# oleg-savchenko/jax_nbody_emulator_with_dj

Hardware: AMD Instinct MI355X
Metric: voxels/sec (disp+vel) on 512^3 box, ndiv=4 (higher is better)
Workload: dtype f32-equivalent: f16x3 split MFMA (3 f16 MFMAs per product, f32 accumulate)

## Files before the change

### jax_nbody_emulator_with_dj_amd/csrc/nbe_kernels_wino.h

```cpp

#ifndef NBE_EPI_MAX
#define NBE_EPI_MAX 1
#endif
#ifndef NBE_WINO_ZROW
#define NBE_WINO_ZROW 1
#endif
#ifndef NBE_WINO_ITEMREG
#define NBE_WINO_ITEMREG 1
#endif
#ifndef NBE_WINO_LOU
#define NBE_WINO_LOU (NBE_XF_F32 ? 0 : 1)
#endif
constexpr int NBE_MAX_WSTAGES = 32;
constexpr int NBE_MAX_WSKIP = 16;
constexpr float WINO_WSCALE = 16384.0f;
constexpr float WINO_WSCALE_F16 = 256.0f;

struct WinoSrc { const char* xa; const char* xb; long dxd; const char* w; long psb; float sb; int pad_; };

struct WinoKArgs {
    int H, W, Dv, Hv, Wv, Ho, Wo;
    int nchunk, cout_groups, flags, ntiles, tny, tnx;
    int zblock;
    float* y; float* dy; long out_pstride; int out_g0;
    const float* bias; const float* gout; const float* beta;
    const float* r; const float* dr; long res_pstride;
    float inv_scale;
    int nskip;
    long dws_delta;
    WinoSrc st[NBE_MAX_WSTAGES + NBE_MAX_WSKIP];
};

template <bool SKIP, bool NOVEL, bool F16 = false>
__global__ __launch_bounds__(512, 2) void conv_h3w_kernel(WinoKArgs a) {
    static_assert(!(F16 && NOVEL), "the float16 form has no displacement-only variant");
    typedef HGGeom<false> G;
    constexpr int NW = 8, CT = 64, TAPU = G::TAPU, WGU = G::WG, XBASE = G::XBASE, MT = 4, NT = 2, NTILE = 8;
    constexpr int ZROW = G::LDS_UNITS;
    f32x4* lds = lds_h3;
    const half8* L8 = (const half8*)lds_h3;
    half8* L8w = (half8*)lds_h3;
    const int tid = threadIdx.x;
    const int lane = tid & 63;
    const int wave = __builtin_amdgcn_readfirstlane(tid >> 6);
    const int c = lane & 15, q = lane >> 4, kh = q & 1, ks = q >> 1;

    const int nct = (a.cout_groups + 7) / 8;
    const int vt = xcd_tile(blockIdx.x, a.ntiles * nct);
    const int tile = vt / nct, ct = vt - tile * nct;
    const int npair = a.Dv >> 1;
    int zp, ty, tx;
    {
        const int zb = a.zblock;
        const int full = (npair / zb) * zb;
        const int per_blk = zb * a.tny * a.tnx;
        if (tile < (npair / zb) * per_blk) {
            const int blk = tile / per_blk, r = tile - blk * per_blk;
            const int zi = r % zb, tyx = r / zb;
            zp = blk * zb + zi; ty = tyx / a.tnx; tx = tyx - ty * a.tnx;
        } else {
            const int r = tile - (npair / zb) * per_blk, rem = npair - full;
            const int zi = r % rem, tyx = r / rem;
            zp = full + zi; ty = tyx / a.tnx; tx = tyx - ty * a.tnx;
        }
    }
    const int y0 = ty * (NOVEL ? 2 * HP_ROWS : HP_ROWS), x0 = tx * HP_COLS, z0 = 2 * zp;
    const int nst = 4 * a.nchunk;

    const long to = (((long)z0 * a.H + y0) * a.W + x0) * 16;
    const long wcm = (long)ct * nst * WGU * 16, wcs = (long)ct * a.nskip * TAPU * 16;

    struct Nxt { const char *xa, *xb, *w0; long dxd, psb; float sb; } nx;
    auto set_next = [&](int s) {
        const WinoSrc e = a.st[s];
        nx.xa = e.xa + to; nx.xb = e.xb + to; nx.dxd = e.dxd; nx.psb = e.psb; nx.w0 = e.w + (SKIP && s >= nst ? wcs : wcm); nx.sb = e.sb;
    };
    unsigned lane16 = (unsigned)lane << 4;
    asm volatile("" : "+v"(lane16));
    auto dma_w = [&](int buf, int t) {
        const int n = wave + NW * t;
        unsigned l16 = (unsigned)lane;
        if (NBE_WINO_ZROW && !F16) l16 = lane16;
        else asm volatile("v_lshlrev_b32 %0, 4, %0" : "+v"(l16));
        if (n < G::NWI) dma16s(nx.w0 + (long)n * 1024, l16, lds + buf * WGU + n * 64);
    };
    auto dma_raw = [&](int buf) {
        unsigned l16 = (unsigned)lane;
        asm volatile("v_lshlrev_b32 %0, 4, %0" : "+v"(l16));
        dma16s(nx.w0 + (wave < 4 ? 0 : a.dws_delta) + (long)(wave & 3) * 1024, l16, lds + buf * WGU + wave * 64);
#pragma unroll
        for (int t = 0; t < 6; ++t) {
            const int tensor = t / 3, n = wave + NW * (t % 3), pl = n / 6, k = n - 6 * pl;
            const int u = k * 64 + lane;
            const int uu = u < HP_PL ? u : HP_PL - 1;
            const int row = (uu * 241) >> 13, col = uu - row * HP_RS;
            if (u < HP_PL)
                dma16s(nx.xa + (tensor ? nx.dxd : 0) + (long)pl * nx.psb, (unsigned)(row * a.W + col) * 16u,
                       lds + XBASE + buf * HQ_XB + tensor * HQ_XT + pl * HQ_PP + k * 64);
        }
    };
    constexpr bool ITEMREG = NBE_WINO_ITEMREG && !F16;
    int it_uu[3] = {0, 0, 0};
    unsigned it_go[3] = {0u, 0u, 0u};
    if (ITEMREG) {
#pragma unroll
        for (int j = 0; j < 3; ++j) {
            const int u = ((wave + NW * j) % 6) * 64 + lane;
            it_uu[j] = u < HP_PL ? u : HP_PL - 1;
            const int row = (it_uu[j] * 241) >> 13, col = it_uu[j] - row * HP_RS;
            it_go[j] = (unsigned)(row * a.W + col) * 16u;
        }
#pragma unroll
        for (int j = 0; j < 3; ++j) asm volatile("" : "+v"(it_uu[j]), "+v"(it_go[j]));
    }
    auto item_unit = [&](int j, bool& valid) {
        if (ITEMREG) {
            valid = lane < HP_PL - ((wave + NW * j) % 6) * 64;
            return it_uu[j];
        }
        int l = lane;
        asm volatile("" : "+v"(l));
        const int u = ((wave + NW * j) % 6) * 64 + l;
        valid = u < HP_PL;
        return valid ? u : HP_PL - 1;
    };
    auto item_goff_j = [&](int j) {
        if (ITEMREG) return it_go[j];
        bool v;
        const int uu = item_unit(j, v);
        const int row = (uu * 241) >> 13, col = uu - row * HP_RS;
        return (unsigned)(row * a.W + col) * 16u;
    };
    typedef unsigned int u32x4 __attribute__((ext_vector_type(4)));
    struct Stg { half8 ah, al, bh, bl; float sb; };
    auto st_load = [&](int j, Stg& g) {
        const int n = wave + NW * j;
        const long po = ((n / 12) ? nx.dxd : 0) + (long)(((n % 12) / 6) * 2) * nx.psb;
        const char* pa = nx.xa + po;
        const char* pb = nx.xb + po;
        const unsigned go = item_goff_j(j);
        const __amdgpu_buffer_rsrc_t ra = __builtin_amdgcn_make_buffer_rsrc((void*)pa, 0, 0xffffffffu, 0x00027000);
        const __amdgpu_buffer_rsrc_t rb = __builtin_amdgcn_make_buffer_rsrc((void*)pb, 0, 0xffffffffu, 0x00027000);
        const unsigned pso = (unsigned)nx.psb;
        auto ld = [&](half8& d, __amdgpu_buffer_rsrc_t r, unsigned so) {
            const u32x4 v = __builtin_amdgcn_raw_buffer_load_b128(r, go, so, 0);
            d = __builtin_bit_cast(half8, v);
        };
        ld(g.ah, ra, 0); ld(g.al, ra, pso); ld(g.bh, rb, 0); ld(g.bl, rb, pso);
        g.sb = nx.sb;
    };
#if NBE_XF_F32
    struct Xf { u32x4 HI, LO; float t0, t1; unsigned h; };
    auto xf_step = [&](const Stg& g, Xf& x, int k) {
        const int r = k >> 2, m = k & 3;
        const unsigned AH = __builtin_bit_cast(u32x4, g.ah)[r], AL = __builtin_bit_cast(u32x4, g.al)[r];
        const unsigned BH = __builtin_bit_cast(u32x4, g.bh)[r], BL = __builtin_bit_cast(u32x4, g.bl)[r];
        const float inv = H3_INV, sinv = g.sb * H3_INV, sb = g.sb, k2048 = H3_SCALE;
        if (m == 0) {
            asm("v_fma_mix_f32 %0, %1, %2, %3 op_sel:[0,0,0] op_sel_hi:[1,0,1]" : "=v"(x.t0) : "v"(AL), "s"(inv), "v"(AH));
            asm("v_fma_mix_f32 %0, %1, %2, %0 op_sel:[0,0,0] op_sel_hi:[1,0,0]" : "+v"(x.t0) : "v"(BL), "s"(sinv));
            asm("v_fma_mix_f32 %0, %1, %2, %0 op_sel:[0,0,0] op_sel_hi:[1,0,0]" : "+v"(x.t0) : "v"(BH), "s"(sb));
        } else if (m == 1) {
            asm("v_fma_mix_f32 %0, %1, %2, %3 op_sel:[1,0,1] op_sel_hi:[1,0,1]" : "=v"(x.t1) : "v"(AL), "s"(inv), "v"(AH));
            asm("v_fma_mix_f32 %0, %1, %2, %0 op_sel:[1,0,0] op_sel_hi:[1,0,0]" : "+v"(x.t1) : "v"(BL), "s"(sinv));
            asm("v_fma_mix_f32 %0, %1, %2, %0 op_sel:[1,0,0] op_sel_hi:[1,0,0]" : "+v"(x.t1) : "v"(BH), "s"(sb));
        } else if (m == 2) {
            asm("v_cvt_pk_f16_f32 %0, %1, %2" : "=v"(x.h) : "v"(x.t0), "v"(x.t1));
            asm("v_fma_mix_f32 %0, %1, -1.0, %0 op_sel:[0,0,0] op_sel_hi:[1,0,0]" : "+v"(x.t0) : "v"(x.h));
            asm("v_fma_mix_f32 %0, %1, -1.0, %0 op_sel:[1,0,0] op_sel_hi:[1,0,0]" : "+v"(x.t1) : "v"(x.h));
        } else {
            unsigned l;
            asm("v_fma_mixlo_f16 %0, %1, %2, 0 op_sel_hi:[0,0,0]" : "=v"(l) : "v"(x.t0), "s"(k2048));
            asm("v_fma_mixhi_f16 %0, %1, %2, 0 op_sel_hi:[0,0,0]" : "+v"(l) : "v"(x.t1), "s"(k2048));
            x.HI[r] = x.h; x.LO[r] = l;
        }
    };
#else
    struct Xf { u32x4 HI, LO; unsigned s, bb, e1, e2, l1; };
    auto xf_step = [&](const Stg& g, Xf& x, int k) {
        const int r = k >> 2, m = k & 3;
        const unsigned AH = __builtin_bit_cast(u32x4, g.ah)[r], AL = __builtin_bit_cast(u32x4, g.al)[r];
        const unsigned BH = __builtin_bit_cast(u32x4, g.bh)[r], BL = __builtin_bit_cast(u32x4, g.bl)[r];
        const unsigned sbp = g.sb < 0.f ? 0xBC00BC00u : 0x3C003C00u, k2048 = 0x68006800u;
        if (F16) {
            if (m == 0) asm("v_pk_fma_f16 %0, %1, %2, %3" : "=v"(x.s) : "v"(BH), "s"(sbp), "v"(AH));
            else if (m == 1) asm("v_pk_fma_f16 %0, %1, %2, %3" : "=v"(x.l1) : "v"(BL), "s"(sbp), "v"(AL));
            else if (m == 3) { x.HI[r] = x.s; x.LO[r] = x.l1; }
            (void)k2048;
        } else
        if (m == 0) {
            asm("v_pk_fma_f16 %0, %1, %2, %3" : "=v"(x.s) : "v"(BH), "s"(sbp), "v"(AH));
            asm("v_pk_add_f16 %0, %1, %2 neg_lo:[0,1] neg_hi:[0,1]" : "=v"(x.bb) : "v"(x.s), "v"(AH));
        } else if (m == 1) {
            asm("v_pk_add_f16 %0, %1, %2 neg_lo:[0,1] neg_hi:[0,1]" : "=v"(x.e1) : "v"(x.s), "v"(x.bb));
            asm("v_pk_fma_f16 %0, %1, %2, %3 neg_lo:[0,0,1] neg_hi:[0,0,1]" : "=v"(x.e2) : "v"(BH), "s"(sbp), "v"(x.bb));
        } else if (m == 2) {
            asm("v_pk_add_f16 %0, %1, %2 neg_lo:[0,1] neg_hi:[0,1]" : "=v"(x.e1) : "v"(AH), "v"(x.e1));
            asm("v_pk_fma_f16 %0, %1, %2, %3" : "=v"(x.l1) : "v"(BL), "s"(sbp), "v"(AL));
        } else {
            unsigned err, l;
            asm("v_pk_add_f16 %0, %1, %2" : "=v"(err) : "v"(x.e1), "v"(x.e2));
#if NBE_WINO_LOU
            const unsigned kinv = 0x10001000u;
            asm("v_pk_fma_f16 %0, %1, %2, %3" : "=v"(l) : "v"(x.l1), "s"(kinv), "v"(err));
            (void)k2048;
#else
            asm("v_pk_fma_f16 %0, %1, %2, %3" : "=v"(l) : "v"(err), "s"(k2048), "v"(x.l1));
#endif
            x.HI[r] = x.s; x.LO[r] = l;
        }
    };
#endif
    auto st_write = [&](int j, int buf, const Xf& x) {
        bool valid;
        const int n = wave + NW * j;
        const int lo_ = XBASE + buf * HQ_XB + (n / 12) * HQ_XT + (((n % 12) / 6) * 2) * HQ_PP + item_unit(j, valid);
        if (valid) {
            L8w[lo_] = __builtin_bit_cast(half8, x.HI);
            L8w[lo_ + HQ_PP] = __builtin_bit_cast(half8, x.LO);
        }
    };
    auto st_store = [&](int j, int buf, Stg& g) {
        Xf x;
#pragma unroll
        for (int k = 0; k < 16; ++k) xf_step(g, x, k);
        st_write(j, buf, x);
    };

    f32x4 YA[NTILE], DA[NTILE], YB[NTILE], DB[NTILE];
#pragma unroll
    for (int t = 0; t < NTILE; ++t)
#pragma unroll
        for (int e = 0; e < 4; ++e) { YA[t][e] = 0.f; DA[t][e] = 0.f; YB[t][e] = 0.f; DB[t][e] = 0.f; }
    auto mm = [&](f32x4& acc, const half8& A, const half8& B) {
        asm("v_mfma_f32_16x16x32_f16 %0, %1, %2, %0" : "+a"(acc) : "v"(A), "v"(B));
    };
    auto mmz = [&](f32x4& acc, const half8& A, const half8& B) {
        asm("s_nop 1\n\tv_mfma_f32_16x16x32_f16 %0, %1, %2, %0" : "+a"(acc) : "v"(A), "v"(B));
    };

    const int rowp = wave;
    const int aP = (ks * 4 + 2 * kh) * CT + c;
    const int bB = (2 * kh) * HQ_PP + rowp * HP_RS + c;
    const int bP1 = bB + ks, bP32 = bB + 32 * ks;
    auto LA = [&](half8 (&r)[MT], int idx) {
#pragma unroll
        for (int mt = 0; mt < MT; ++mt) r[mt] = L8[idx + 16 * mt];
    };
    auto LB = [&](half8 (&r)[NT], int idx) {
#pragma unroll
        for (int nt = 0; nt < NT; ++nt) r[nt] = L8[idx + 16 * nt];
    };
    const _Float16 kInv = (_Float16)H3_INV;
#define SNAKE(i) ((((i) >> 1) & 1) ? ((i) ^ 1) : (i))
    auto nohook = [](int) {};
    auto MM8h = [&](f32x4 (&acc)[NTILE], const half8 (&A)[MT], const half8 (&B)[NT], int slot, int nb, bool px, bool zsel,
                    bool hooked, auto&& hook) {
#pragma unroll
        for (int i = 0; i < NTILE; ++i) {
            const int t = SNAKE(i);
            if (zsel && (i % NT) == 0) mmz(acc[t], A[t / NT], B[t % NT]); else
            mm(acc[t], A[t / NT], B[t % NT]);
            if (hooked) { hook(i); __builtin_amdgcn_sched_barrier(0); }
            if (slot >= 0 && (i % 4) == 3) {
                if (px) dma_w(nb, slot + i / 4);
                __builtin_amdgcn_sched_barrier(0);
            }
        }
    };
    auto MM8 = [&](f32x4 (&acc)[NTILE], const half8 (&A)[MT], const half8 (&B)[NT], int slot, int nb, bool px, bool zsel = false) {
        MM8h(acc, A, B, slot, nb, px, zsel, false, nohook);
    };
    auto MM8s = [&](f32x4 (&acc)[NTILE], half8 (&P)[MT], const half8 (&A)[MT], const half8 (&B)[NT], int slot, int nb, bool px) {
        P[0] = A[0] * kInv;
#pragma unroll
        for (int i = 0; i < NTILE; ++i) {
            const int t = SNAKE(i);
            if ((i % NT) == 0) { if (t / NT + 1 < MT) P[t / NT + 1] = A[t / NT + 1] * kInv; mmz(acc[t], P[t / NT], B[t % NT]); }
            else mm(acc[t], P[t / NT], B[t % NT]);
            if (slot >= 0 && (i % 4) == 3) {
                if (px) dma_w(nb, slot + i / 4);
                __builtin_amdgcn_sched_barrier(0);
            }
        }
    };
#define NBE_SB __builtin_amdgcn_sched_barrier(0)
    half8 wh[MT], wl[MT], wp[MT], xh[NT], xl[NT], dxh[NT], dxl[NT];
    auto pair = [&](f32x4 (&Y)[NTILE], f32x4 (&DY)[NTILE], int slot0, int nb, bool px, int wa, int xp,
                    auto&& preXl, auto&& preW, auto&& preXh, auto&& mid, bool hooked, auto&& hook, auto&& after3) {
        if (F16) {
            LB(dxh, xp + HQ_XT); LA(wl, wa + CT + aP);
            NBE_SB; MM8h(Y, wh, xh, slot0, nb, px, false, hooked, [&](int t) { hook(t); }); NBE_SB;
            LB(dxl, xp + HQ_XT + HQ_PP);
            NBE_SB; MM8h(Y, wl, xl, slot0 < 0 ? -1 : slot0 + 2, nb, px, false, hooked, [&](int t) { hook(8 + t); }); NBE_SB;
            after3();
            mid();
            preXl(); preXh();
            NBE_SB; MM8(DY, wh, dxh, slot0 < 0 ? -1 : slot0 + 4, nb, px); NBE_SB;
            preW();
            NBE_SB; MM8(DY, wl, dxl, -1, nb, px); NBE_SB;
            return;
        }
        LB(dxh, xp + HQ_XT);
#if NBE_WINO_LOU
        NBE_SB; MM8(Y, wh, xl, slot0, nb, px); NBE_SB;
#else
        NBE_SB; MM8s(Y, wp, wh, xl, slot0, nb, px); NBE_SB;
#endif
        LB(dxl, xp + HQ_XT + HQ_PP);
        NBE_SB; MM8h(Y, wh, xh, slot0 < 0 ? -1 : slot0 + 2, nb, px, false, hooked, [&](int t) { hook(t); }); NBE_SB;
        LA(wl, wa + CT + aP);
        NBE_SB; MM8h(DY, wh, dxh, slot0 < 0 ? -1 : slot0 + 4, nb, px, false, hooked, [&](int t) { hook(8 + t); }); NBE_SB;
        after3();
        mid();
#if NBE_WINO_LOU
        NBE_SB; MM8(DY, wh, dxl, -1, nb, px); NBE_SB;
#else
        NBE_SB; MM8(DY, wp, dxl, -1, nb, px); NBE_SB;
#endif
        preXl(); preW();
        NBE_SB; MM8(Y, wl, xh, -1, nb, px); NBE_SB;
        preXh();
        NBE_SB; MM8(DY, wl, dxh, -1, nb, px); NBE_SB;
    };

    constexpr int SH4 = HP_RS + 1, SH5 = HP_RS + 2, SH7 = 2 * HP_RS + 1;
    auto stage = [&](f32x4 (&Y)[NTILE], f32x4 (&DY)[NTILE], int s, auto nxt) {
        constexpr int NXT = decltype(nxt)::value;
        constexpr bool px = NXT == 1;
        const bool pre = px && s + 1 != 2 * a.nchunk;
        if (NXT) set_next(s + 1);
        int par = s & 1;
        asm volatile("" : "+s"(par));
        int nb = 1 - par;
        asm volatile("" : "+s"(nb));
        const int wb = par * WGU, xb = XBASE + par * HQ_XB;
        const int wbn = nb * WGU, xbn = XBASE + nb * HQ_XB;
        Stg g;
        Xf xf;
        auto hk = [&](int k) { xf_step(g, xf, k); };
        auto none = [] {};
        if (NXT == 2) dma_raw(nb);
        if (px) st_load(0, g);
        pair(Y, DY, 0, nb, px, wb, xb + bP1,
             [&] { LB(xl, xb + 2 + bP32 + HQ_PP); }, [&] { LA(wh, wb + 2 * TAPU + aP); }, [&] { LB(xh, xb + 2 + bP32); },
             none, false, nohook, none);
        half8 a1[MT], a2[MT], b1x[NT], b1d[NT];
        const int aS = wb + 4 * TAPU + (2 * kh + (F16 ? ks : 0)) * CT + c;
        const int bS = xb + (2 * kh + ks) * HQ_PP + rowp * HP_RS + c + SH4;
        pair(Y, DY, -1, nb, px, wb + 2 * TAPU, xb + 2 + bP32,
             [&] { LB(b1x, bS); }, [&] { LA(a1, aS); }, [&] { LB(b1d, bS + HQ_XT); }, none,
             px, hk, [&] { if (px) { st_write(0, nb, xf); st_load(1, g); } });
        const half8 zero = {0, 0, 0, 0, 0, 0, 0, 0};
        if (F16) {
            NBE_SB; MM8(Y, a1, b1x, -1, 0, false); NBE_SB;
            LB(xl, xb + SH5 + bP32 + HQ_PP); LB(xh, xb + SH5 + bP32); LA(wh, wb + 5 * TAPU + aP);
            NBE_SB; MM8(DY, a1, b1d, -1, 0, false); NBE_SB;
        } else {
#if NBE_WINO_LOU
        NBE_SB; MM8(Y, a1, b1x, -1, 0, false); NBE_SB;
#else
        {
            const _Float16 m1 = ks ? kInv : (_Float16)1.0f;
#pragma unroll
            for (int mt = 0; mt < MT; ++mt) a1[mt] = a1[mt] * m1;
        }
        NBE_SB; MM8(Y, a1, b1x, -1, 0, false, true); NBE_SB;
#endif
#if NBE_WINO_ZROW
        LA(a2, ks ? ZROW + c : aS + CT);
#else
        LA(a2, aS + CT);
#endif
        LB(xl, xb + SH5 + bP32 + HQ_PP);
        NBE_SB; MM8(DY, a1, b1d, -1, 0, false); NBE_SB;
        LB(xh, xb + SH5 + bP32); LA(wh, wb + 5 * TAPU + aP);
#if NBE_WINO_ZROW
        NBE_SB; MM8(Y, a2, b1x, -1, 0, false); NBE_SB;
#else
#pragma unroll
        for (int mt = 0; mt < MT; ++mt) a2[mt] = ks ? zero : a2[mt];
        NBE_SB; MM8(Y, a2, b1x, -1, 0, false, true); NBE_SB;
#endif
        MM8(DY, a2, b1d, -1, 0, false); NBE_SB;
        }
        pair(Y, DY, -1, nb, px, wb + 5 * TAPU, xb + SH5 + bP32,
             [&] { LB(xl, xb + SH7 + bP1 + HQ_PP); }, [&] { LA(wh, wb + 7 * TAPU + aP); }, [&] { LB(xh, xb + SH7 + bP1); },
             none, px, hk, [&] { if (px) { st_write(1, nb, xf); st_load(2, g); } });
        pair(Y, DY, -1, nb, px, wb + 7 * TAPU, xb + SH7 + bP1,
             [&] { if (pre) LB(xl, xbn + bP1 + HQ_PP); }, [&] { if (pre) LA(wh, wbn + aP); }, [&] { if (pre) LB(xh, xbn + bP1); },
             [&] { asm volatile("s_waitcnt vmcnt(0) lgkmcnt(0)\n\ts_barrier" ::: "memory"); },
             px, hk, [&] { if (px) st_write(2, nb, xf); });
    };

    auto raw_stage = [&](f32x4 (&Y)[NTILE], f32x4 (&DY)[NTILE], int s, bool px) {
        if (px) set_next(s + 1);
        int par = s & 1;
        asm volatile("" : "+s"(par));
        int nb = 1 - par;
        asm volatile("" : "+s"(nb));
        const int wb = par * WGU, xb = XBASE + par * HQ_XB;
        if (px) dma_raw(nb);
        half8 a1[MT], a2[MT], d1[MT], d2[MT], bx[NT], bd[NT];
        const half8 zero = {0, 0, 0, 0, 0, 0, 0, 0};
        const _Float16 m1 = ks ? kInv : (_Float16)1.0f;
        const int aS = wb + (2 * kh) * CT + c;
        const int bS = xb + (2 * kh + ks) * HQ_PP + rowp * HP_RS + c + SH4;
        if (F16) {
            const int aF = wb + (2 * kh + ks) * CT + c;
            LA(a1, aF); LB(bx, bS); LB(bd, bS + HQ_XT); LA(d1, aF + TAPU);
            NBE_SB; MM8(Y, a1, bx, -1, 0, false); NBE_SB;
            MM8(DY, a1, bd, -1, 0, false); NBE_SB;
            MM8(DY, d1, bx, -1, 0, false); NBE_SB;
            asm volatile("s_waitcnt vmcnt(0) lgkmcnt(0)\n\ts_barrier" ::: "memory");
            return;
        }
        LA(a1, aS); LB(bx, bS); LA(a2, aS + CT); LB(bd, bS + HQ_XT);
#pragma unroll
        for (int mt = 0; mt < MT; ++mt) a1[mt] = a1[mt] * m1;
        NBE_SB; MM8(Y, a1, bx, -1, 0, false, true); NBE_SB;
        if (!NOVEL) LA(d1, aS + TAPU);
#pragma unroll
        for (int mt = 0; mt < MT; ++mt) a2[mt] = ks ? zero : a2[mt];
        NBE_SB; MM8(Y, a2, bx, -1, 0, false, true); NBE_SB;
        if (!NOVEL) LA(d2, aS + TAPU + CT);
        if (NOVEL || !(a.flags & F_SKIP_NODX)) {
            NBE_SB; MM8(DY, a1, bd, -1, 0, false); NBE_SB;
            MM8(DY, a2, bd, -1, 0, false); NBE_SB;
        }
        if (!NOVEL) {
#pragma unroll
            for (int mt = 0; mt < MT; ++mt) { d1[mt] = d1[mt] * m1; d2[mt] = ks ? zero : d2[mt]; }
            NBE_SB; MM8(DY, d1, bx, -1, 0, false, true); NBE_SB;
            MM8(DY, d2, bx, -1, 0, false, true); NBE_SB;
        }
        asm volatile("s_waitcnt vmcnt(0) lgkmcnt(0)\n\ts_barrier" ::: "memory");
    };

    {
        if (NBE_WINO_ZROW && !F16 && tid < 64) L8w[ZROW + tid] = half8{0, 0, 0, 0, 0, 0, 0, 0};
        set_next(0);
#pragma unroll
        for (int k = 0; k < G::NWS; ++k) dma_w(0, k);
        {
            Stg g0, g1, g2;
            st_load(0, g0); st_load(1, g1); st_load(2, g2);
            st_store(0, 0, g0); st_store(1, 0, g1); st_store(2, 0, g2);
        }
        asm volatile("s_waitcnt vmcnt(0) lgkmcnt(0)" ::: "memory");
        __syncthreads();
        LA(wh, aP); LB(xl, XBASE + bP1 + HQ_PP); LB(xh, XBASE + bP1);
    }

    auto butterfly = [&] {
            asm volatile("s_nop 15\n\ts_nop 15" ::: "memory");
#pragma unroll
            for (int t = 0; t < NTILE; ++t) {
                f32x4 p, m;
#pragma unroll
                for (int e = 0; e < 4; ++e) { p[e] = acc_read(YA[t][e]); m[e] = acc_read(YB[t][e]); }
                YA[t] = p + m; YB[t] = p - m;
                asm volatile("" : "+a"(YA[t]), "+a"(YB[t]));
                __builtin_amdgcn_sched_barrier(0);
#pragma unroll
                for (int e = 0; e < 4; ++e) { p[e] = acc_read(DA[t][e]); m[e] = acc_read(DB[t][e]); }
                DA[t] = p + m; DB[t] = p - m;
                asm volatile("" : "+a"(DA[t]), "+a"(DB[t]));
                __builtin_amdgcn_sched_barrier(0);
            }
            asm volatile("s_nop 7" ::: "memory");
            LA(wh, aP); LB(xl, XBASE + bP1 + HQ_PP); LB(xh, XBASE + bP1);
    };
    const int npairs = 2 * a.nchunk;
    for (int s2 = 0; s2 + 1 < npairs; ++s2) {
        if (s2 == a.nchunk) butterfly();
        stage(YA, DA, 2 * s2, std::integral_constant<int, 1>());
        stage(YB, DB, 2 * s2 + 1, std::integral_constant<int, 1>());
    }
    if (npairs - 1 == a.nchunk) butterfly();
    stage(YA, DA, 2 * npairs - 2, std::integral_constant<int, 1>());
    stage(YB, DB, 2 * npairs - 1, std::integral_constant<int, SKIP ? 2 : 0>());
    if (SKIP) {
        for (int sc = 0; sc < a.nskip; ++sc) {
            raw_stage(YA, DA, nst + 2 * sc, true);
            raw_stage(YB, DB, nst + 2 * sc + 1, sc + 1 < a.nskip);
        }
    }
#undef NBE_SB
#undef SNAKE
    asm volatile("s_nop 15\n\ts_nop 15" ::: "memory");

    const bool act = a.flags & F_ACT, gauge = !NOVEL && a.gout != nullptr;
    f32x4 bv[MT], be[MT], gv[MT];
    int unit[MT];
    bool uok[MT];
#pragma unroll
    for (int mt = 0; mt < MT; ++mt) {
        unit[mt] = ct * (CT / 8) + 2 * mt + ks;
        uok[mt] = unit[mt] < a.cout_groups;
        if (!uok[mt]) unit[mt] = a.cout_groups - 1;
        bv[mt] = *(const f32x4*)(a.bias + unit[mt] * 8 + 4 * kh);
        be[mt] = f32x4{0.f, 0.f, 0.f, 0.f};
        if (!NOVEL) be[mt] = *(const f32x4*)(a.beta + unit[mt] * 8 + 4 * kh);
        gv[mt] = f32x4{0.f, 0.f, 0.f, 0.f};
        if (!NOVEL && gauge) gv[mt] = *(const f32x4*)(a.gout + unit[mt] * 8 + 4 * kh);
    }
#pragma unroll
    for (int mt = 0; mt < MT; ++mt) asm volatile("" : "+v"(bv[mt]), "+v"(be[mt]), "+v"(gv[mt]));
    long ob_mt[MT];
#pragma unroll
    for (int mt = 0; mt < MT; ++mt) ob_mt[mt] = (long)(a.out_g0 + (F16 ? 1 : 2) * unit[mt]) * a.out_pstride * 16 + 8 * kh;
    const long ol_off = a.out_pstride * 16;
    auto epilogue = [&](f32x4 (&Y)[NTILE], f32x4 (&DY)[NTILE], int z) {
        int o[NT];
        bool ook[NT], ook2[NT];
#pragma unroll
        for (int nt = 0; nt < NT; ++nt) {
            const int yy = y0 + rowp, xx = x0 + 16 * nt + c;
            ook[nt] = yy < a.Hv && xx < a.Wv;
            ook2[nt] = NOVEL && yy + HP_ROWS < a.Hv && xx < a.Wv;
            o[nt] = ook[nt] ? (z * a.Ho + yy) * a.Wo + xx : z * a.Ho * a.Wo;
        }
        half4 r0[F16 ? NTILE : 1], r1[F16 ? NTILE : 1];
        const bool res = F16 && (a.flags & F_RES);
        if (F16 && res) {
#pragma unroll
            for (int t = 0; t < NTILE; ++t) {
                const int mt = t / NT, nt = t % NT;
                const long rb = ((long)unit[mt] * a.res_pstride + (long)o[nt]) * 16 + 8 * kh;
                r0[t] = *(const half4*)((const char*)a.r + rb);
                r1[t] = *(const half4*)((const char*)a.dr + rb);
            }
#pragma unroll
            for (int t = 0; t < NTILE; ++t) asm volatile("" : "+v"(r0[t]), "+v"(r1[t]));
        }
#pragma unroll
        for (int mt = 0; mt < MT; ++mt) {
#pragma unroll
            for (int nt = 0; nt < NT; ++nt) {
                const int t = mt * NT + nt;
                f32x4 v, dv;
                __builtin_amdgcn_sched_barrier(0);
#pragma unroll
                for (int e = 0; e < 4; ++e) {
                    const float yp = acc_read(Y[t][e]) * a.inv_scale;
                    v[e] = yp + bv[mt][e];
                    dv[e] = acc_read(DY[t][e]) * a.inv_scale + be[mt][e] * yp;
                }
                if (F16 && res) {
#pragma unroll
                    for (int e = 0; e < 4; ++e) { v[e] += (float)r0[t][e]; dv[e] += (float)r1[t][e]; }
                }
                if (act) {
#pragma unroll
                    for (int e = 0; e < 4; ++e) {
                        dv[e] = v[e] > 0.f ? dv[e] : 0.01f * dv[e];
                        v[e] = (F16 || !NBE_EPI_MAX) ? (v[e] >= 0.f ? v[e] : 0.01f * v[e]) : __builtin_fmaxf(v[e], 0.01f * v[e]);
                    }
                }
                if (gauge) {
#pragma unroll
                    for (int e = 0; e < 4; ++e) dv[e] += gv[mt][e] * v[e];
                }
                if (F16) {
                    if (uok[mt] && ook[nt]) {
                        const long ob = ob_mt[mt] + (long)o[nt] * 16;
                        half4 h, dh;
#pragma unroll
                        for (int e = 0; e < 4; ++e) { h[e] = (_Float16)v[e]; dh[e] = (_Float16)dv[e]; }
                        *(half4*)((char*)a.y + ob) = h;
                        *(half4*)((char*)a.dy + ob) = dh;
                    }
                } else
                if (NOVEL) {
#pragma unroll
                    for (int e = 0; e < 4; ++e) {
                        dv[e] = acc_read(DY[t][e]) * a.inv_scale + bv[mt][e];
                        if (act) dv[e] = dv[e] >= 0.f ? dv[e] : 0.01f * dv[e];
                    }
                    const long ob = ob_mt[mt] + (long)o[nt] * 16;
                    const long ol = ob + ol_off;
                    const long r8 = (long)HP_ROWS * a.Wo * 16;
                    half4 hi, lo;
                    if (uok[mt] && ook[nt]) {
                        split4(v, hi, lo);
                        *(half4*)((char*)a.y + ob) = hi;
                        *(half4*)((char*)a.y + ol) = lo;
                    }
                    if (uok[mt] && ook2[nt]) {
                        split4(dv, hi, lo);
                        *(half4*)((char*)a.y + ob + r8) = hi;
                        *(half4*)((char*)a.y + ol + r8) = lo;
                    }
                } else
                if (uok[mt] && ook[nt]) {
                    const long ob = ob_mt[mt] + (long)o[nt] * 16;
                    const long ol = ob + ol_off;
                    half4 hi, lo;
                    split4(v, hi, lo);
                    *(half4*)((char*)a.y + ob) = hi;
                    *(half4*)((char*)a.y + ol) = lo;
                    split4(dv, hi, lo);
                    *(half4*)((char*)a.dy + ob) = hi;
                    *(half4*)((char*)a.dy + ol) = lo;
                }
            }
        }
    };
    epilogue(YA, DA, z0);
    epilogue(YB, DB, z0 + 1);
}

__global__ __launch_bounds__(256) void pack_h3w_kernel(const float* __restrict__ w, int cout, int cin, int nchunk, long total,
                                                       _Float16* __restrict__ dst, int* __restrict__ flag, int f16) {
    const long idx = (long)blockIdx.x * blockDim.x + threadIdx.x;
    if (idx >= total) return;
    long r = idx;
    const int j = (int)(r % 8); r /= 8;
    const int co = (int)(r % 64); r /= 64;
    const int u = (int)(r % 4); r /= 4;
    const int tap = (int)(r % 9); r /= 9;
    const int stage = (int)(r % (4 * nchunk)); r /= 4 * nchunk;
    const int ct = (int)r;
    const int chunk = stage >> 2, xi = stage & 3;
    const int h = u >> 1, part = u & 1;
    const int ci = f16 ? chunk * 32 + 8 * u + j : chunk * 16 + 8 * h + j, oc = ct * 64 + co;
    float v = 0.f;
    if (oc < cout && ci < cin) {
        const float* p = w + (((size_t)oc * cin + ci) * 3) * 9 + tap;
        const float w0 = p[0], w1 = p[9], w2 = p[18];
        v = xi == 0 ? w0 : xi == 1 ? 0.5f * (w0 + w1 + w2) : xi == 2 ? 0.5f * (w0 - w1 + w2) : -w2;
    }
    v *= f16 ? WINO_WSCALE_F16 : WINO_WSCALE;
    if (!(fabsf(v) <= 60000.f)) { atomicOr(flag, 1); v = 0.f; }
    const _Float16 hi = (_Float16)v;
    dst[idx] = (part == 0 || f16) ? hi : (_Float16)(v - (float)hi);
}

void launch_pack_h3w(const float* w_oidhw, int cout, int cin, int cin_pad, int ctiles, float* dst, int* flag, hipStream_t s, int prec) {
    const bool f16 = prec == PREC_F16;
    const int nchunk = cin_pad / (f16 ? 32 : 16);
    const long total = (long)ctiles * 4 * nchunk * 9 * 4 * 64 * 8;
    hipLaunchKernelGGL(pack_h3w_kernel, dim3((unsigned)((total + 255) / 256)), dim3(256), 0, s, w_oidhw, cout, cin, nchunk, total,
                       (_Float16*)dst, flag, f16 ? 1 : 0);
}

static int launch_h3w(const ConvKArgs& ka_in, const float* ww, const float* wws, long wws_set_floats, int ctiles, hipStream_t s,
                      bool novel = false, bool f16 = false) {
    typedef HGGeom<false> G;
    constexpr size_t smem = (size_t)(G::LDS_UNITS + 64) * 16;
    static_assert(smem <= 160 * 1024, "LDS budget of one CU");
    ConvKArgs ka = ka_in;
    if (f16) {
        if (novel || (ka.nchunk & 1) || (ka.csplit < ka.nchunk && (ka.csplit & 1))) return 1;
        if (ka.nskip > 0 && ((ka.nskip & 1) || (ka.s_csplit < ka.nskip && (ka.s_csplit & 1)) || (ka.flags & F_SKIP_NODX))) return 1;
        ka.nchunk /= 2; if (ka.csplit < (1 << 29)) ka.csplit /= 2;
        ka.nskip /= 2; if (ka.s_csplit < (1 << 29)) ka.s_csplit /= 2;
    }
    if (!ww || (!f16 && (ka.flags & F_RES)) || (ka.Dv & 1) || 4 * ka.nchunk > NBE_MAX_WSTAGES || (!novel && !ka.beta)) return 1;
    if (ka.nskip > 0 && (!wws || 2 * ka.nskip > NBE_MAX_WSKIP)) return 1;
    if (ctiles != (ka.cout_groups + 7) / 8) return 1;
    if (std::max(ka.in_pstride, ka.csplit < ka.nchunk ? ka.in2_pstride : 0L) * 16 + 16L * (HP_ROWS + 2) * ka.W >= (1L << 32) - (1L << 20)) return 1;
    WinoKArgs wa;
    wa.H = ka.H; wa.W = ka.W; wa.Dv = ka.Dv; wa.Hv = ka.Hv; wa.Wv = ka.Wv; wa.Ho = ka.Ho; wa.Wo = ka.Wo;
    wa.nchunk = ka.nchunk; wa.cout_groups = ka.cout_groups; wa.flags = ka.flags;
    const int trows = novel ? 2 * HP_ROWS : HP_ROWS;
    wa.tny = (ka.Hv + trows - 1) / trows;
    wa.tnx = (ka.Wv + HP_COLS - 1) / HP_COLS;
    wa.ntiles = (ka.Dv / 2) * wa.tny * wa.tnx;
    wa.y = ka.y; wa.dy = ka.dy; wa.out_pstride = ka.out_pstride; wa.out_g0 = ka.out_g0;
    wa.bias = ka.bias; wa.gout = novel ? nullptr : ka.gout; wa.beta = novel ? nullptr : ka.beta;
    const long rows8 = (long)HP_ROWS * ka.W * 16;
    wa.inv_scale = 1.0f / (f16 ? WINO_WSCALE_F16 : WINO_WSCALE);
    wa.r = ka.r; wa.dr = ka.dr; wa.res_pstride = ka.res_pstride;
    wa.zblock = std::min(8, ka.Dv / 2);
    wa.nskip = ka.nskip; wa.dws_delta = wws_set_floats * 4;
    static const int XI[2][2] = {{1, 2}, {0, 3}};
    static const int PA[4] = {0, 1, 2, 1}, PB[4] = {2, 2, 1, 3};
    static const float SB[4] = {-1.f, 1.f, -1.f, -1.f};
    const long plane = (long)ka.H * ka.W * 16;
    for (int ph = 0; ph < 2; ++ph)
        for (int chunk = 0; chunk < ka.nchunk; ++chunk)
            for (int ab = 0; ab < 2; ++ab) {
                const int xi = XI[ph][ab];
                const bool second = chunk >= ka.csplit;
                const long ps = second ? ka.in2_pstride : ka.in_pstride;
                const char* x = (const char*)(second ? ka.x2 : ka.x);
                const char* dx = (const char*)(second ? ka.dx2 : ka.dx);
                const long off = (long)(second ? chunk - ka.csplit : chunk) * 4 * ps * 16;
                WinoSrc& e = wa.st[(ph * ka.nchunk + chunk) * 2 + ab];
                e.xa = x + off + PA[xi] * plane; e.xb = x + off + PB[xi] * plane; e.dxd = novel ? rows8 : dx - x;
                e.w = (const char*)ww + (long)(chunk * 4 + xi) * G::WG * 16; e.psb = ps * 16; e.sb = SB[xi]; e.pad_ = 0;
            }
    for (int sc = 0; sc < ka.nskip; ++sc)
        for (int ab = 0; ab < 2; ++ab) {
            const bool second = sc >= ka.s_csplit;
            const long ps = second ? ka.s2_pstride : ka.s_pstride;
            const char* x = (const char*)(second ? ka.xs2 : ka.xs);
            const char* dx = (const char*)(second ? ka.dxs2 : ka.dxs);
            const long off = (long)(second ? sc - ka.s_csplit : sc) * 4 * ps * 16 + ab * plane;
            WinoSrc& e = wa.st[4 * ka.nchunk + 2 * sc + ab];
            e.xa = x + off; e.xb = e.xa; e.dxd = novel ? rows8 : dx - x; e.w = (const char*)wws + (long)sc * G::TAPU * 16; e.psb = ps * 16; e.sb = 0.f; e.pad_ = 0;
        }
    const bool skip = ka.nskip > 0;
    if (novel) wa.dws_delta = 0;
    auto kern = f16 ? (skip ? conv_h3w_kernel<true, false, true> : conv_h3w_kernel<false, false, true>)
              : novel ? (skip ? conv_h3w_kernel<true, true> : conv_h3w_kernel<false, true>)
              : (skip ? conv_h3w_kernel<true, false> : conv_h3w_kernel<false, false>);
    ensure_lds_limit((const void*)kern, smem);
    dim3 grid(wa.ntiles * ctiles, 1, 1), block(512, 1, 1);
    hipLaunchKernelGGL(kern, grid, block, smem, s, wa);
    return 0;
}
```

Baseline: 101.5 million.

## Stage skip-conv weights in idle LDS once and stream activations to registers

For the non-float16 path, the skip (raw) stages stop running one DMA-plus-barrier round per chunk. Instead, all skip-chunk weights are loaded once into the now idle weight and activation LDS buffers. The skip activations are read straight from global memory into double-buffered registers, one chunk ahead, and the MFMA chain runs across all skip chunks without block barriers. This aims to remove per-chunk synchronisation and LDS round-trips in the skip tail, at the cost of more VGPRs and uncoalesced direct global loads.

```diff
diff --git a/jax_nbody_emulator_with_dj_amd/csrc/nbe_kernels_wino.h b/jax_nbody_emulator_with_dj_amd/csrc/nbe_kernels_wino.h
--- a/jax_nbody_emulator_with_dj_amd/csrc/nbe_kernels_wino.h
+++ b/jax_nbody_emulator_with_dj_amd/csrc/nbe_kernels_wino.h
@@ -73,7 +73,7 @@
     struct Nxt { const char *xa, *xb, *w0; long dxd, psb; float sb; } nx;
     auto set_next = [&](int s) {
         const WinoSrc e = a.st[s];
-        nx.xa = e.xa + to; nx.xb = e.xb + to; nx.dxd = e.dxd; nx.psb = e.psb; nx.w0 = e.w + (SKIP && s >= nst ? wcs : wcm); nx.sb = e.sb;
+        nx.xa = e.xa + to; nx.xb = e.xb + to; nx.dxd = e.dxd; nx.psb = e.psb; nx.w0 = e.w + (SKIP && F16 && s >= nst ? wcs : wcm); nx.sb = e.sb;
     };
     unsigned lane16 = (unsigned)lane << 4;
     asm volatile("" : "+v"(lane16));
@@ -99,6 +99,29 @@
                        lds + XBASE + buf * HQ_XB + tensor * HQ_XT + pl * HQ_PP + k * 64);
         }
     };
+    constexpr int SKU = 2 * TAPU;
+    static_assert(4 * SKU <= WGU && (NBE_MAX_WSKIP / 2 - 4) * SKU <= HQ_XB, "the skip's weights fit the idle buffer pair");
+    auto sk_wbase = [&](int sc) { return sc < 4 ? sc * SKU : XBASE + (sc - 4) * SKU; };
+    auto sk_weights = [&] {
+        unsigned l16 = (unsigned)lane;
+        asm volatile("v_lshlrev_b32 %0, 4, %0" : "+v"(l16));
+        const char* w = a.st[nst].w + wcs + (wave < 4 ? 0 : a.dws_delta) + (long)(wave & 3) * 1024;
+        for (int sc = 0; sc < a.nskip; ++sc) dma16s(w + (long)sc * (TAPU * 16), l16, lds + sk_wbase(sc) + wave * 64);
+    };
+    struct SkB { half8 x[2][NT], d[2][NT]; };
+    const bool sk_dx = NOVEL || !(a.flags & F_SKIP_NODX);
+    auto sk_load = [&](SkB& b, int sc) {
+#pragma unroll
+        for (int ab = 0; ab < 2; ++ab) {
+            const WinoSrc& e = a.st[nst + 2 * sc + ab];
+            const char* p = e.xa + to + ((long)(2 * kh + ks) * e.psb + (long)(((wave + 1) * a.W + c + 1) * 16));
+#pragma unroll
+            for (int nt = 0; nt < NT; ++nt) b.x[ab][nt] = *(const half8*)(p + 256 * nt);
+#pragma unroll
+            for (int nt = 0; nt < NT; ++nt) b.d[ab][nt] = *(const half8*)(p + e.dxd + 256 * nt);
+        }
+    };
+    SkB skP, skQ;
     constexpr bool ITEMREG = NBE_WINO_ITEMREG && !F16;
     int it_uu[3] = {0, 0, 0};
     unsigned it_go[3] = {0u, 0u, 0u};
@@ -329,7 +352,7 @@
         constexpr int NXT = decltype(nxt)::value;
         constexpr bool px = NXT == 1;
         const bool pre = px && s + 1 != 2 * a.nchunk;
-        if (NXT) set_next(s + 1);
+        if (NXT == 1 || (NXT == 2 && F16)) set_next(s + 1);
         int par = s & 1;
         asm volatile("" : "+s"(par));
         int nb = 1 - par;
@@ -340,7 +363,8 @@
         Xf xf;
         auto hk = [&](int k) { xf_step(g, xf, k); };
         auto none = [] {};
-        if (NXT == 2) dma_raw(nb);
+        if (NXT == 2 && F16) dma_raw(nb);
+        if (NXT == 2 && !F16) { sk_weights(); sk_load(skP, 0); NBE_SB; }
         if (px) st_load(0, g);
         pair(Y, DY, 0, nb, px, wb, xb + bP1,
              [&] { LB(xl, xb + 2 + bP32 + HQ_PP); }, [&] { LA(wh, wb + 2 * TAPU + aP); }, [&] { LB(xh, xb + 2 + bP32); },
@@ -401,40 +425,62 @@
         asm volatile("" : "+s"(nb));
         const int wb = par * WGU, xb = XBASE + par * HQ_XB;
         if (px) dma_raw(nb);
-        half8 a1[MT], a2[MT], d1[MT], d2[MT], bx[NT], bd[NT];
-        const half8 zero = {0, 0, 0, 0, 0, 0, 0, 0};
-        const _Float16 m1 = ks ? kInv : (_Float16)1.0f;
-        const int aS = wb + (2 * kh) * CT + c;
+        half8 a1[MT], d1[MT], bx[NT], bd[NT];
         const int bS = xb + (2 * kh + ks) * HQ_PP + rowp * HP_RS + c + SH4;
-        if (F16) {
-            const int aF = wb + (2 * kh + ks) * CT + c;
-            LA(a1, aF); LB(bx, bS); LB(bd, bS + HQ_XT); LA(d1, aF + TAPU);
-            NBE_SB; MM8(Y, a1, bx, -1, 0, false); NBE_SB;
-            MM8(DY, a1, bd, -1, 0, false); NBE_SB;
-            MM8(DY, d1, bx, -1, 0, false); NBE_SB;
-            asm volatile("s_waitcnt vmcnt(0) lgkmcnt(0)\n\ts_barrier" ::: "memory");
-            return;
-        }
-        LA(a1, aS); LB(bx, bS); LA(a2, aS + CT); LB(bd, bS + HQ_XT);
-#pragma unroll
-        for (int mt = 0; mt < MT; ++mt) a1[mt] = a1[mt] * m1;
-        NBE_SB; MM8(Y, a1, bx, -1, 0, false, true); NBE_SB;
-        if (!NOVEL) LA(d1, aS + TAPU);
-#pragma unroll
-        for (int mt = 0; mt < MT; ++mt) a2[mt] = ks ? zero : a2[mt];
-        NBE_SB; MM8(Y, a2, bx, -1, 0, false, true); NBE_SB;
-        if (!NOVEL) LA(d2, aS + TAPU + CT);
-        if (NOVEL || !(a.flags & F_SKIP_NODX)) {
-            NBE_SB; MM8(DY, a1, bd, -1, 0, false); NBE_SB;
-            MM8(DY, a2, bd, -1, 0, false); NBE_SB;
+        const int aF = wb + (2 * kh + ks) * CT + c;
+        LA(a1, aF); LB(bx, bS); LB(bd, bS + HQ_XT); LA(d1, aF + TAPU);
+        NBE_SB; MM8(Y, a1, bx, -1, 0, false); NBE_SB;
+        MM8(DY, a1, bd, -1, 0, false); NBE_SB;
+        MM8(DY, d1, bx, -1, 0, false); NBE_SB;
+        asm volatile("s_waitcnt vmcnt(0) lgkmcnt(0)\n\ts_barrier" ::: "memory");
+    };
+
+    const _Float16 skm1 = ks ? kInv : (_Float16)1.0f;
+    const half8 zero8 = {0, 0, 0, 0, 0, 0, 0, 0};
+    auto sk_hi = [&](int wb_) { LA(wh, wb_ + (2 * kh) * CT + c); };
+    auto sk_lo = [&](int wb_) {
+        if (NBE_WINO_ZROW) LA(wl, ks ? ZROW + c : wb_ + (2 * kh + 1) * CT + c);
+        else LA(wl, wb_ + (2 * kh + 1) * CT + c);
+    };
+    auto sk_scale = [&] {
+#pragma unroll
+        for (int mt = 0; mt < MT; ++mt) wh[mt] = wh[mt] * skm1;
+    };
+    auto sk_zero = [&] {
+        if (NBE_WINO_ZROW) return;
+#pragma unroll
+        for (int mt = 0; mt < MT; ++mt) wl[mt] = ks ? zero8 : wl[mt];
+    };
+    auto sk_chunk = [&](const SkB& b, SkB& bn, int sc, int ld) {
+        const bool more = ld >= 0;
+        const int wb_ = sk_wbase(sc), wbn_ = sk_wbase(sc + 1);
+        if (more) sk_load(bn, ld);
+        sk_scale();
+        NBE_SB; MM8(YA, wh, b.x[0], -1, 0, false, true); NBE_SB;
+        MM8(YB, wh, b.x[1], -1, 0, false); NBE_SB;
+        if (sk_dx) {
+            MM8(DA, wh, b.d[0], -1, 0, false); NBE_SB;
+            MM8(DB, wh, b.d[1], -1, 0, false); NBE_SB;
+        }
+        if (!NOVEL) sk_hi(wb_ + TAPU); else if (more) sk_hi(wbn_);
+        sk_zero();
+        NBE_SB; MM8(YA, wl, b.x[0], -1, 0, false, !NBE_WINO_ZROW); NBE_SB;
+        MM8(YB, wl, b.x[1], -1, 0, false); NBE_SB;
+        if (sk_dx) {
+            MM8(DA, wl, b.d[0], -1, 0, false); NBE_SB;
+            MM8(DB, wl, b.d[1], -1, 0, false); NBE_SB;
         }
         if (!NOVEL) {
-#pragma unroll
-            for (int mt = 0; mt < MT; ++mt) { d1[mt] = d1[mt] * m1; d2[mt] = ks ? zero : d2[mt]; }
-            NBE_SB; MM8(DY, d1, bx, -1, 0, false, true); NBE_SB;
-            MM8(DY, d2, bx, -1, 0, false, true); NBE_SB;
-        }
-        asm volatile("s_waitcnt vmcnt(0) lgkmcnt(0)\n\ts_barrier" ::: "memory");
+            sk_lo(wb_ + TAPU);
+            sk_scale();
+            NBE_SB; MM8(DA, wh, b.x[0], -1, 0, false, true); NBE_SB;
+            MM8(DB, wh, b.x[1], -1, 0, false); NBE_SB;
+            if (more) sk_hi(wbn_);
+            sk_zero();
+            NBE_SB; MM8(DA, wl, b.x[0], -1, 0, false, !NBE_WINO_ZROW); NBE_SB;
+            MM8(DB, wl, b.x[1], -1, 0, false); NBE_SB;
+        }
+        if (more) sk_lo(wbn_);
     };
 
     {
@@ -480,11 +526,22 @@
     if (npairs - 1 == a.nchunk) butterfly();
     stage(YA, DA, 2 * npairs - 2, std::integral_constant<int, 1>());
     stage(YB, DB, 2 * npairs - 1, std::integral_constant<int, SKIP ? 2 : 0>());
-    if (SKIP) {
+    if (SKIP && F16) {
         for (int sc = 0; sc < a.nskip; ++sc) {
             raw_stage(YA, DA, nst + 2 * sc, true);
             raw_stage(YB, DB, nst + 2 * sc + 1, sc + 1 < a.nskip);
         }
+    }
+    if (SKIP && !F16) {
+        sk_hi(sk_wbase(0));
+        sk_lo(sk_wbase(0));
+        __builtin_amdgcn_s_waitcnt(0x0F70);
+        int sc = 0;
+        for (; sc + 1 < a.nskip; sc += 2) {
+            sk_chunk(skP, skQ, sc, sc + 1);
+            sk_chunk(skQ, skP, sc + 1, sc + 2 < a.nskip ? sc + 2 : sc + 1);
+        }
+        if (sc < a.nskip) sk_chunk(skP, skQ, sc, -1);
     }
 #undef NBE_SB
 #undef SNAKE
```

After: 102.7 million, median of 6. 1.3% higher.
